# Tarekbouamer/Image-Retrieval-for-Image-Based-Localization

Measured on AMD Instinct MI355X. Metric: images/sec extract + queries/sec 1M-desc kNN, ResNet50-GeM 1024×768, higher is better.
Workload: dtype fp16

## Files before the change

### image-retrieval-for-image-based-localization_amd/cirtorch/_engine.py

```python

import contextlib
import ctypes
import os
import threading

import torch

PKG_DIR = os.path.dirname(os.path.dirname(os.path.abspath(__file__)))
LIB_PATH = os.environ.get("RR_LIB", os.path.join(PKG_DIR, "librr.so"))

RR_F32, RR_BF16, RR_F16, RR_I8 = 0, 1, 2, 3
RR_ACT_IDENTITY, RR_ACT_LEAKY = 0, 1
RR_POOL_GEM, RR_POOL_MAC, RR_POOL_SPOC = 0, 1, 2
RR_CONV_AFFINE, RR_CONV_RESIDUAL, RR_CONV_PERM32 = 1, 2, 4
RR_NHWC, RR_NCHW = 0, 1
RR_MATCH_NN, RR_MATCH_MNN, RR_MATCH_SNN, RR_MATCH_SMNN = 0, 1, 2, 3
RR_RESP_HARRIS, RR_RESP_GFTT, RR_RESP_HESSIAN, RR_RESP_DOG = 0, 1, 2, 3
RR_EPI_SAMPSON, RR_EPI_SYMMETRICAL = 0, 1
TUNE_KEYS = ("GEMM_CONFIG", "GEMM_STAGES", "GEMM_WIDE", "GEMM_ASTAT", "GEMM_XCD_MAP", "STREAM_1X1", "CONV3X3",
             "GRID_CUS", "GEMM8", "KNN_FUSED", "CONV3_PIPE", "STEM", "STREAM_XCD", "CONV3S", "WRES", "PAIR_MID",
             "WRES_RING")
globals().update(("RR_TUNE_" + name, key) for key, name in enumerate(TUNE_KEYS))
TUNE_SIZE_KEYS = {"PATCHNET_CHUNK": 32}
globals().update(("RR_TUNE_" + name, key) for name, key in TUNE_SIZE_KEYS.items())
RR_PATCHNET_HARDNET, RR_PATCHNET_SOSNET = 0, 1

_DTYPE_CODE = {torch.float32: RR_F32, torch.bfloat16: RR_BF16, torch.float16: RR_F16,
               torch.int8: RR_I8}


class ConvDesc(ctypes.Structure):
    _fields_ = [(n, ctypes.c_int) for n in ("n", "h", "w", "c_in", "ho", "wo", "c_out", "kh", "kw", "stride",
                                            "pad", "dil", "k_packed", "ldy", "act")] + \
               [("slope", ctypes.c_float), ("flags", ctypes.c_int)]


class LaunchInfo(ctypes.Structure):
    _fields_ = [("kernel", ctypes.c_char * 32), ("variant", ctypes.c_char * 48), ("grid", ctypes.c_uint),
                ("block", ctypes.c_uint), ("nslices", ctypes.c_int), ("xmap", ctypes.c_int), ("launches", ctypes.c_int)]


class Region(ctypes.Structure):
    _fields_ = [(n, ctypes.c_uint16) for n in ("y0", "x0", "h", "w")]


_vp, _i, _ll, _f, _d, _sz = ctypes.c_void_p, ctypes.c_int, ctypes.c_longlong, ctypes.c_float, ctypes.c_double, ctypes.c_size_t
_SIGS = {
    "rr_version": ([], _i),
    "rr_build_info": ([], ctypes.c_char_p),
    "rr_last_error": ([], ctypes.c_char_p),
    "rr_device_arch": ([ctypes.c_char_p, _i], _i),
    "rr_image_to_nhwc": ([_vp, _i, _i, _i, _i, ctypes.POINTER(_f), ctypes.POINTER(_f), _i, _vp, _i, _i, _vp], _i),
    "rr_conv2d_fused": ([_vp, _vp, _vp, _vp, _vp, _vp, ctypes.POINTER(ConvDesc), _i, _i, _vp], _i),
    "rr_conv1x1_pair": ([_vp, _ll, _i, _vp, _vp, _vp, _i, _vp, _vp, _vp, _vp, _vp, _i, _f, _vp, _vp, _vp, _i, _i, _f,
                         _vp, _vp, _i, _vp], _i),
    "rr_conv3x3_pair": ([_vp, _i, _i, _i, _vp, _vp, _vp, _i, _f, _vp, _vp, _vp, _i, _f, _vp, _vp, _vp, _vp, _vp, _vp, _vp, _vp, _i, _f,
                         _vp, _vp, _vp, _i, _i, _f, _vp, _vp, _vp, _i, _vp], _i),
    "rr_pack_conv_weights": ([_vp, _i, _i, _i, _i, _i, _i, _i, _vp, _i, _vp], _i),
    "rr_stem_pack_weights": ([_vp, _i, _i, _i, _i, _vp, _i, _vp], _i),
    "rr_stem_conv_pool": ([_vp, _i, _i, _i, ctypes.POINTER(_f), ctypes.POINTER(_f), _i, _vp, _vp, _vp, _i, _f, _vp,
                           _i, _i, _i, _vp], _i),
    "rr_stem_conv_pool_u8": ([_vp, _i, _i, _i, ctypes.POINTER(_f), ctypes.POINTER(_f), _i, _vp, _vp, _vp, _i, _f,
                              _vp, _i, _i, _i, _vp], _i),
    "rr_image_to_nhwc_ragged": ([_vp, _vp, _i, _i, _i, _i, _i, ctypes.POINTER(_f), ctypes.POINTER(_f), _i, _vp, _i,
                                 _i, _vp], _i),
    "rr_stem_conv_pool_ragged": ([_vp, _vp, _i, _i, _i, _i, ctypes.POINTER(_f), ctypes.POINTER(_f), _i, _vp, _vp, _vp,
                                  _i, _f, _vp, _i, _i, _i, _vp], _i),
    "rr_pad_images": ([_vp, _vp, _i, _i, _i, _i, _i, _vp, _vp, _vp], _i),
    "rr_maxpool2d": ([_vp, _i, _i, _i, _i, _i, _i, _i, _vp, _i, _i, _i, _vp], _i),
    "rr_resize_bilinear": ([_vp, _i, _i, _i, _vp, _i, _i, _d, _d, _vp], _i),
    "rr_global_pool": ([_vp, _i, _i, _i, _i, _i, _f, _f, _vp, _i, _vp], _i),
    "rr_global_pool_pdev": ([_vp, _i, _i, _i, _i, _i, _f, _vp, _f, _vp, _i, _vp], _i),
    "rr_region_pool": ([_vp, _i, _i, _i, _i, ctypes.POINTER(Region), _i, _i, _f, _vp, _i, _f, _vp, _i, _vp], _i),
    "rr_region_aggregate": ([_vp, _i, _i, _i, _i, _f, _vp, _vp], _i),
    "rr_l2n_rows": ([_vp, _i, _i, _f, _vp, _vp], _i),
    "rr_linear_rows": ([_vp, _i, _i, _vp, _vp, _i, _vp, _vp], _i),
    "rr_head_workspace_bytes": ([_i, _i], _sz),
    "rr_whiten_workspace_bytes": ([_i, _i], _sz),
    "rr_whitenapply": ([_vp, _i, _i, _vp, _vp, _i, _vp, _vp, _sz, _vp], _i),
    "rr_head_l2n_whiten_l2n": ([_vp, _i, _i, _vp, _vp, _i, _f, _vp, _vp, _vp], _i),
    "rr_knn_workspace_bytes": ([_ll, _i, _i, _i, _i, _i], _sz),
    "rr_knn_topk": ([_vp, _vp, _ll, _vp, _vp, _i, _i, _i, _i, _ll, _vp, _vp, _vp, _sz, _i, _vp], _i),
    "rr_knn_topk_checked": ([_vp, _vp, _ll, _vp, _vp, _i, _i, _i, _i, _ll, _vp, _vp, _vp, _sz, _i, _f, _vp, _vp], _i),
    "rr_topk_merge": ([_vp, _vp, _i, _i, _i, _i, _vp, _vp, _vp], _i),
    "rr_comm_unique_id": ([_vp, _i], _i),
    "rr_comm_init": ([ctypes.POINTER(_vp), _i, _vp, _i, _i], _i),
    "rr_comm_destroy": ([_vp], _i),
    "rr_topk_allgather_workspace_bytes": ([_i, _i, _i], _sz),
    "rr_topk_allgather_merge": ([_vp, _vp, _vp, _i, _i, _vp, _vp, _vp, _sz, _vp], _i),
    "rr_local_head_workspace_bytes": ([_ll, _i, _i], _sz),
# ... 182 lines not shown
```

### image-retrieval-for-image-based-localization_amd/cirtorch/_ops.py

```python

import ctypes
import os

import numpy as np
import torch

from . import _engine as E


def _st():
    return E.stream_ptr()


def _workspace(nbytes, device):
    return torch.empty(max(int(nbytes), 256), dtype=torch.uint8, device=device)


def image_to_nhwc(img, c_pad, dtype, mean=None, std=None):
    E.require_gpu(img)
    img = img.contiguous().float()
    n, c, h, w = img.shape
    out = torch.empty((n, h, w, c_pad), dtype=dtype, device=img.device)
    do = mean is not None
    m = (ctypes.c_float * 4)(*(list(mean) + [0.0] * (4 - c))[:4]) if do else (ctypes.c_float * 4)()
# ... 49 lines not shown
        return torch.empty(shape_y, dtype=dtype, device=device), torch.empty(shape_z, dtype=dtype, device=device)
    y, z = out
    E.require_gpu(y, z)
    assert tuple(y.shape) == shape_y and y.dtype == dtype and y.is_contiguous()
    assert tuple(z.shape) == shape_z and z.dtype == dtype and z.is_contiguous()
    return y, z


def conv1x1_pair(x, w3, scale3, shift3, residual, leaky3, slope3, w1, scale1, shift1, c_out, leaky1, slope1,
                 proj=None, out=None):
    E.require_gpu(x, w3, residual, w1)
    n, h, w, c = x.shape
    c_mid = w3.shape[0]
    y, z = _pair_out(out, (n, h, w, c_mid), (n, h, w, c_out), x.dtype, x.device)
    assert x.is_contiguous()
    if residual is not None:
        assert residual.shape == y.shape and residual.dtype == x.dtype and residual.is_contiguous()
        xp = wp = sp = hp = None
    else:
        xp, wp, sp, hp = proj
        E.require_gpu(xp, wp, sp, hp)
        assert xp.shape == x.shape and xp.dtype == x.dtype and xp.is_contiguous()
    E.check(E.lib().rr_conv1x1_pair(E.ptr(x), n * h * w, c, E.ptr(w3), E.ptr(scale3), E.ptr(shift3), c_mid,
                                    E.ptr(residual), E.ptr(xp), E.ptr(wp), E.ptr(sp), E.ptr(hp),
                                    E.RR_ACT_LEAKY if leaky3 else E.RR_ACT_IDENTITY, float(slope3),
                                    E.ptr(w1), E.ptr(scale1), E.ptr(shift1), c_out,
                                    E.RR_ACT_LEAKY if leaky1 else E.RR_ACT_IDENTITY, float(slope1), E.ptr(y), E.ptr(z),
                                    E.dtype_code(x.dtype), _st()), "rr_conv1x1_pair")
    return y, z


def conv3x3_pair(t1, w33, scale2, shift2, leaky2, slope2, w3, scale3, shift3, residual, leaky3, slope3,
                 w1, scale1, shift1, c_out, leaky1, slope1, proj=None, dynamic=None, conv1=None,
                 out=None):
    E.require_gpu(t1, w33, w3, residual, w1)
    n, h, w, c = t1.shape
    assert c == 64 and t1.is_contiguous() and tuple(w33.shape) == (64, 576) and tuple(w3.shape) == (256, 64)
    assert tuple(w1.shape) == (c_out, 256)
    y, z = _pair_out(out, (n, h, w, 256), (n, h, w, c_out), t1.dtype, t1.device)
    if residual is not None:
        assert residual.shape == y.shape and residual.dtype == t1.dtype and residual.is_contiguous()
        xp = wp = sp = hp = None
    else:
        xp, wp, sp, hp = proj
        E.require_gpu(xp, wp, sp, hp)
        assert tuple(xp.shape) == (n, h, w, 64) and xp.dtype == t1.dtype and xp.is_contiguous()
    act = lambda leaky: E.RR_ACT_LEAKY if leaky else E.RR_ACT_IDENTITY
    if dynamic is None:
        dynamic = os.environ.get("RR_C3PAIR_QUEUE", "1") != "0"
    queue = torch.zeros(8, dtype=torch.int32, device=t1.device) if dynamic else None
    w0, s0, h0, leaky0, slope0 = conv1 if conv1 is not None else (None, None, None, False, 0.0)
    if conv1 is not None:
        E.require_gpu(w0, s0, h0)
        assert proj is not None and tuple(w0.shape) == (64, 64)
    E.check(E.lib().rr_conv3x3_pair(E.ptr(t1), n, h, w, E.ptr(w0), E.ptr(s0), E.ptr(h0), act(leaky0), float(slope0),
                                    E.ptr(w33), E.ptr(scale2), E.ptr(shift2), act(leaky2),
                                    float(slope2), E.ptr(w3), E.ptr(scale3), E.ptr(shift3), E.ptr(residual),
                                    E.ptr(xp), E.ptr(wp), E.ptr(sp), E.ptr(hp), act(leaky3), float(slope3),
                                    E.ptr(w1), E.ptr(scale1), E.ptr(shift1), c_out, act(leaky1), float(slope1),
                                    E.ptr(y), E.ptr(z), E.ptr(queue), E.dtype_code(t1.dtype), _st()),
            "rr_conv3x3_pair")
    return y, z


def maxpool2d(x, k=3, stride=2, pad=1):
    E.require_gpu(x)
    n, h, w, c = x.shape
    ho = (h + 2 * pad - k) // stride + 1
    wo = (w + 2 * pad - k) // stride + 1
    y = torch.empty((n, ho, wo, c), dtype=x.dtype, device=x.device)
    E.check(E.lib().rr_maxpool2d(E.ptr(x), n, h, w, c, k, stride, pad, E.ptr(y), ho, wo, E.dtype_code(x.dtype),
                                 _st()), "rr_maxpool2d")
    return y


def pack_stem_weights(weight, dtype=torch.bfloat16):
    E.require_gpu(weight)
    w = weight.detach().float().contiguous()
    co, ci, kh, kw = w.shape
    out = torch.empty((co, 448), dtype=dtype, device=w.device)
    E.check(E.lib().rr_stem_pack_weights(E.ptr(w), co, ci, kh, kw, E.ptr(out), E.dtype_code(dtype), _st()),
            "rr_stem_pack_weights")
    return out


_UNIT_LUT = {}


def pixels_to_unit(x):
    lut = _UNIT_LUT.get(x.device)
    if lut is None:
        lut = torch.from_numpy(np.arange(256, dtype=np.float32) / np.float32(255.0)).to(x.device)
        _UNIT_LUT[x.device] = lut
    return lut[x.long()]
# ... 1211 lines not shown
```

### image-retrieval-for-image-based-localization_amd/cirtorch/backbones/resnet.py

```python

import os
import sys
from collections import OrderedDict
from functools import partial

import torch
import torch.nn as nn
import torch.nn.functional as F

from .. import _ops
from ..modules.abn import ABN
from .misc import ResidualBlock, make_step, run_step

CONV_PARAMS = ["weight"]
BN_PARAMS = ["weight", "bias", "running_mean", "running_var"]

_PRECISIONS = {"bf16": torch.bfloat16, "fp32": torch.float32, "float32": torch.float32, "bfloat16": torch.bfloat16,
               "fp16": torch.float16, "float16": torch.float16}


def try_index(scalar_or_list, i):
    try:
        return scalar_or_list[i]
    except TypeError:
# ... 115 lines not shown
            for blk in mod.children():
                blocks.append(blk.engine_plan(self.engine_dtype))
            plan["mods"].append(blocks)
        self._plan = plan
        return plan

    @staticmethod
    def _conv(t, st, residual=None, out=None):
        return run_step(t, st, residual, out)

    def _stem(self, plan, x, mean, std):
        if isinstance(x, (list, tuple)):
            live = [t for t in x if t is not None]
            if not live:
                raise ValueError("at least one image of the batch must be non-None")
            h = max(int(t.shape[-2]) for t in live)
            w = max(int(t.shape[-1]) for t in live)
            st = plan["stem"]
            if plan["stem_fused"] is not None:
                return _ops.stem_conv_pool_ragged(x, h, w, plan["stem_fused"], st.scale, st.shift, leaky=st.leaky,
                                                  slope=st.slope, mean=mean, std=std)
            t = _ops.image_to_nhwc_ragged(x, h, w, self.stem_cin(), self.engine_dtype, mean, std)
            return _ops.maxpool2d(self._conv(t, st), 3, 2, 1)
        if x.dtype == torch.uint8 and plan["stem_fused"] is None:
            x = _ops.pixels_to_unit(x)
        if plan["stem_fused"] is not None:
            st = plan["stem"]
            return _ops.stem_conv_pool(x, plan["stem_fused"], st.scale, st.shift, leaky=st.leaky, slope=st.slope,
                                       mean=mean, std=std)
        t = _ops.image_to_nhwc(x, self.stem_cin(), self.engine_dtype, mean, std)
        t = self._conv(t, plan["stem"])
        return _ops.maxpool2d(t, 3, 2, 1)

    def _blocks(self, t, flat, i0, i1, outs, pending=None):
        for i in range(i0, i1):
            mod_id, steps, proj = flat[i]
            nxt = flat[i + 1][1][0] if i + 1 < i1 else None
            pair = self._pairable(steps[-1], nxt)
            fuse_proj = pair and proj is not None and self._proj_fusable(proj)
            res = t if proj is None else (None if fuse_proj else self._conv(t, proj))
            block = pair and self._c3pairable(t, steps, nxt, fuse_proj)
            conv1 = block and fuse_proj and pending is None and self._conv1_fusable(t, steps[0])
            y = t
            for j, st in enumerate(steps[:-2] if block else steps[:-1]):
                if conv1:
                    break
                y = pending if (j == 0 and pending is not None) else self._conv(y, st)
            pending = None
            if block:
                mid, last = steps[-2], steps[-1]
                c1 = steps[0]
                t, pending = _ops.conv3x3_pair(y, mid.w, mid.scale, mid.shift, mid.leaky, mid.slope,
                                               last.w, last.scale, last.shift, res, last.leaky, last.slope,
                                               nxt.w, nxt.scale, nxt.shift, nxt.c_out, nxt.leaky, nxt.slope,
                                               proj=(t, proj.w, proj.scale, proj.shift) if fuse_proj else None,
                                               conv1=(c1.w, c1.scale, c1.shift, c1.leaky, c1.slope) if conv1 else None)
            elif pair:
                last = steps[-1]
                t, pending = _ops.conv1x1_pair(y, last.w, last.scale, last.shift, res, last.leaky, last.slope,
                                               nxt.w, nxt.scale, nxt.shift, nxt.c_out, nxt.leaky, nxt.slope,
                                               proj=(t, proj.w, proj.scale, proj.shift) if fuse_proj else None)
            else:
                t = self._conv(y, steps[-1], residual=res)
            if outs is not None and (i + 1 == len(flat) or flat[i + 1][0] != mod_id):
                outs["mod%d" % (mod_id + 2)] = t
        return t, pending

    def forward(self, x, normalize=None):
        plan = self._plan or self._build_plan()
        mean, std = normalize if normalize is not None else (None, None)
        outs = OrderedDict()
        flat = [(mod_id, steps, proj) for mod_id, blocks in enumerate(plan["mods"]) for steps, proj in blocks]
        t = self._stem(plan, x, mean, std)
        outs["mod1"] = t
        self._blocks(t, flat, 0, len(flat), outs)
        return OrderedDict((k, v.permute(0, 3, 1, 2)) for k, v in outs.items())

    @staticmethod
    def _proj_fusable(proj):
        return (proj.kh == 1 and proj.stride == 1 and proj.pad == 0 and proj.perm and proj.c_out == 256
                and proj.w.shape[1] == 64 and not proj.leaky)

    @staticmethod
    def _c3pairable(t, steps, nxt, fuse_proj):
        if len(steps) != 3 or os.environ.get("RR_C3PAIR", "1") == "0":
            return False
        mid, last = steps[1], steps[2]
        n, h, w, c = t.shape
        return (mid.kh == 3 and mid.kw == 3 and mid.stride == 1 and mid.pad == 1 and mid.perm and mid.c_out == 64
                and tuple(mid.w.shape) == (64, 576) and last.c_out == 256 and last.w.shape[1] == 64
                and nxt.c_out in ((64,) if fuse_proj else (64, 128)) and h % 4 == 0 and w % 32 == 0
                and n * h * w * 64 * 2 < 2 ** 31)

    @staticmethod
    def _conv1_fusable(t, st):
        return (os.environ.get("RR_C3PAIR_CONV1", "0") == "1" and st.kh == 1 and st.kw == 1 and st.stride == 1
                and st.pad == 0 and st.perm and st.c_out == 64 and tuple(st.w.shape) == (64, 64) and t.shape[-1] == 64)

    def _pairable(self, last, nxt):
        if nxt is None or self.engine_dtype == torch.float32 or os.environ.get("RR_PAIR_FUSED", "1") == "0":
            return False
        if not (last.kh == 1 and last.stride == 1 and last.perm and nxt.kh == 1 and nxt.stride == 1
                and nxt.pad == 0 and nxt.perm):
            return False
        if last.c_out == 256 and last.w.shape[1] == 64:
            return nxt.w.shape[1] == 256 and nxt.c_out in (64, 128)
        if last.c_out == 512 and last.w.shape[1] == 128 and os.environ.get("RR_PAIR_MID", "1") != "0":
            return nxt.w.shape[1] == 512 and nxt.c_out == 128
        return False
# ... 16 lines not shown
```

### image-retrieval-for-image-based-localization_amd/cirtorch/models/GF_net.py

```python

import os
from collections import OrderedDict

import numpy as np
import torch
import torch.nn as nn

from .. import _ops
from ..algos.GF_algo import globalFeatureAlgo
from ..backbones import resnet as _resnet
from ..modules.heads.global_head import globalHead
from ..modules.pools import POOLING_LAYERS
from ..utils.parallel import PackedSequence

from ..modules.utils import OUTPUT_DIM


class Normalize:

    def __init__(self, rgb_mean=(0.485, 0.456, 0.406), rgb_std=(0.229, 0.224, 0.225)):
        self.rgb_mean = list(rgb_mean)
        self.rgb_std = list(rgb_std)


# ... 10 lines not shown
        out = []
        for scale in scales:
            if scale == 1:
                out.append(img)
            else:
                out.append(PackedSequence([_ops.resize_bilinear(im, scale) for im in img]))
        return out

    def _normalizer(self):
        a = self.augment
        if a is None:
            return None
        if hasattr(a, "rgb_mean") and hasattr(a, "rgb_std"):
            return (list(a.rgb_mean), list(a.rgb_std))
        raise NotImplementedError("only normalising augment objects (rgb_mean/rgb_std) are supported at eval time")

    @property
    def pool(self):
        return self.ret_head.pool

    def meta_repr(self):
        tmp = "  (meta): dict( \n"
        for k in ("architecture", "local_whitening", "pooling", "regional", "whitening", "outputdim", "mean", "std"):
            if k in self.meta:
                tmp += "     %s: %s\n" % (k, self.meta[k])
        tmp += "  )\n"
        return tmp

    def forward(self, img=None, positive_img=None, negative_img=None, scales=[1], do_augmentaton=False,
                do_loss=False, do_prediction=True, **varargs):
        if do_loss:
            raise NotImplementedError("training (tuple loss) is out of scope for the MI355X engine")
        if isinstance(img, torch.Tensor) and img.dim() == 4 and len(scales) == 1:
            x = self.body(img, normalize=self._normalizer())
            ret_pred = self.ret_algo.inference(self.ret_head, x, [img.shape[-2:]] * img.shape[0]) \
                if do_prediction else None
            return OrderedDict([("ret_loss", None)]), OrderedDict([("ret_pred", ret_pred)])
        if isinstance(img, torch.Tensor) and img.dim() == 4:
            preds = []
            for scale in scales:
                if scale == 1:
                    xs = img
                else:
                    xf = _ops.pixels_to_unit(img) if img.dtype == torch.uint8 else img
                    xs = _ops.resize_bilinear(xf, scale)
                _, pred = self.forward(img=xs, scales=[1], do_prediction=True, do_loss=False)
                preds.append(pred["ret_pred"].unsqueeze(0))
            pred = torch.cat(preds, dim=0).permute(1, 2, 0)
            pred = nn.functional.avg_pool1d(pred, kernel_size=len(scales)).squeeze(-1)
            return OrderedDict([("ret_loss", None)]), OrderedDict([("ret_pred", pred)])
        if isinstance(img, torch.Tensor):
            if img.dtype == torch.uint8 and len(scales) > 1:
                img = _ops.pixels_to_unit(img)
            img = PackedSequence(list(img)) if img.dim() == 4 else PackedSequence([img])
        if len(scales) > 1:
            if img.dtype == torch.uint8:
                img = PackedSequence([_ops.pixels_to_unit(t) if t is not None else None for t in img])
            preds = []
            for im in self._prepare_pyramid_inputs(img, scales):
                _, pred = self.forward(img=im, scales=[1], do_prediction=True, do_loss=False)
                preds.append(pred["ret_pred"].unsqueeze(0))
            pred = torch.cat(preds, dim=0).permute(1, 2, 0)
            pred = nn.functional.avg_pool1d(pred, kernel_size=len(scales)).squeeze(-1)
            return OrderedDict([("ret_loss", None)]), OrderedDict([("ret_pred", pred)])

        images = list(img)
        x = self.body(images, normalize=self._normalizer())
        valid_size = [tuple(t.shape[-2:]) if t is not None else (0, 0) for t in images]
        if do_prediction:
            ret_pred = self.ret_algo.inference(self.ret_head, x, valid_size)
        else:
            ret_pred = None
        return OrderedDict([("ret_loss", None)]), OrderedDict([("ret_pred", ret_pred)])

    def extract(self, images, scales=(1,)):
        if not isinstance(images, torch.Tensor):
            images = PackedSequence(list(images))
        with torch.no_grad():
            _, pred = self.forward(img=images, scales=list(scales))
        return pred["ret_pred"]


def make_net(architecture="resnet50", pooling="gem", whitening=True, mean=None, std=None, precision="bf16",
             p=3.0, regional=False, regional_whitening=True, L=3):
    body = _resnet.__dict__[architecture](precision=precision)
    dim = OUTPUT_DIM[architecture]
    pname = {"gem": "GeM", "mac": "MAC", "spoc": "SPoC", "gemmp": "GeMmp"}[pooling.lower()]
    params = {"p": p, "eps": 1e-6} if pname in ("GeM", "GeMmp") else {}
    if regional:
        if pname == "GeMmp":
            params["mp"] = dim
        rwhiten = nn.Linear(dim, dim, bias=True) if regional_whitening else None
        params = {"rpool": POOLING_LAYERS[pname](**params), "whiten": rwhiten, "L": L}
        pname = "ROIpool"
    head = globalHead(pooling={"name": pname, "params": params}, normal={"name": "L2N", "params": {}}, dim=dim)
    algo = globalFeatureAlgo(loss=None, min_level=0, fpn_levels=1)
    if not whitening:
        algo._head = lambda h, x: h(x, do_whitening=False)
    augment = Normalize(mean, std) if mean is not None else None
    net = ImageRetrievalNet(body, algo, head, augment=augment)
# ... 316 lines not shown
```

### image-retrieval-for-image-based-localization_amd/csrc/rr_c3pair.hip

```cpp
#include "rr_internal.h"
#include "rr_ldsdma.h"
#include "rr_epilogue.h"
#include "rr_tilewalk.h"

#ifndef C3P_IG2
#define C3P_IG2 1
#endif

namespace rr {

namespace {

template <int K>
__device__ __forceinline__ int cwswz(int row, int chunk) {
    const int f = K == 64 ? ((row >> 1) & 7) : (row & 15);
    return row * (K * 2) + ((chunk ^ f) << 4);
}

}

struct C3PairArgs {
    const bf16_t* t1;
    const bf16_t* w0;
    const float *s0, *h0;
    const bf16_t* w33;
    const float *s33, *h33;
    const bf16_t* w3;
    const float *s3, *h3;
    const bf16_t* res;
    const bf16_t* xp;
    const bf16_t* wp;
    const float *sp, *hp;
    const bf16_t* w1;
    const float *s1, *h1;
    bf16_t* y;
    bf16_t* z;
    int* queue;
    int n, h, w;
    int act2, act3, act1, act0;
    float slope2, slope3, slope1, slope0;
};

namespace {

template <int C1, bool PROJ, typename HT, bool CONV1 = false>
__global__ void __launch_bounds__(512, 1) k_c3pair(C3PairArgs a, int tiles_w, int tiles_hw, int ntiles) {
    static_assert(!CONV1 || PROJ, "conv1 in the launch: the stage's first block only");
    constexpr int TH = 4, TW = 32, TP = TH * TW, PITCH = 40;
    constexpr int NSLOT = (TH + 2) * PITCH, NP = NSLOT / 8;
    constexpr int PCW = TW + 2;
    constexpr int FN = 4;
    constexpr int K3 = 64, C3 = 256, NK3 = K3 / 32, NR3 = C3 / 32, NF1 = C1 / 16, NK1 = C3 / 32;
    static_assert(NSLOT % 8 == 0 && PITCH % 8 == 0, "row-invariant patch swizzle");
    __shared__ __attribute__((aligned(1024))) char sPatch[NSLOT * 128];
    __shared__ __attribute__((aligned(16))) char sT2[TP * 128];
    __shared__ __attribute__((aligned(16))) char sW3[C3 * K3 * 2];
    __shared__ __attribute__((aligned(16))) char sW1[C1 * C3 * 2];
    __shared__ __attribute__((aligned(16))) char sWp[PROJ ? C3 * K3 * 2 : 16];
    __shared__ __attribute__((aligned(16))) float sS3[C3], sH3[C3], sS1[C1], sH1[C1], sS2[64], sH2[64];
    __shared__ __attribute__((aligned(16))) float sSp[PROJ ? C3 : 4], sHp[PROJ ? C3 : 4];
    __shared__ __attribute__((aligned(16))) char sW0[CONV1 ? 64 * 64 * 2 : 16];
    __shared__ __attribute__((aligned(16))) float sS0[CONV1 ? 64 : 4], sH0[CONV1 ? 64 : 4];
    __shared__ int sTile[4];

    const int tid = threadIdx.x, lane = tid & 63;
    const int wave = __builtin_amdgcn_readfirstlane(tid >> 6);
    const bool role3 = wave < 4;
    const int r16 = lane & 15, kq = lane >> 4, lrow = lane >> 3, lch = lane & 7;
    const int H = a.h, W = a.w;

    for (int i = tid; i < C3 * K3 / 8; i += 512) {
        const int r = i / (K3 / 8), c = i - r * (K3 / 8);
        *reinterpret_cast<uint4*>(sW3 + cwswz<K3>(r, c)) = reinterpret_cast<const uint4*>(a.w3)[i];
        if constexpr (PROJ) *reinterpret_cast<uint4*>(sWp + cwswz<K3>(r, c)) = reinterpret_cast<const uint4*>(a.wp)[i];
    }
    for (int i = tid; i < C1 * C3 / 8; i += 512) {
        const int r = i / (C3 / 8), c = i - r * (C3 / 8);
        *reinterpret_cast<uint4*>(sW1 + cwswz<C3>(r, c)) = reinterpret_cast<const uint4*>(a.w1)[i];
    }
    for (int i = tid; i < C3; i += 512) {
// ... 145 lines not shown
        }
        const bool leaky2 = a.act2 == RR_ACT_LEAKY;
#pragma unroll
        for (int j = 0; j < FN; ++j) {
            const int p = wpx * (TP / 2) + j * 16 + r16;
            float v[8];
            RR_BN_PAIR(acc[0][j], acc[1][j], sc, sh, v);
            if (leaky2) RR_LEAKY(8, v, a.slope2);
            uint4 o;
            RR_PACK8(HT, o, v);
            *reinterpret_cast<uint4*>(sT2 + p * 128 + (((4 * wc + kq) ^ (p & 7)) << 4)) = o;
        }
    };

    const int pw = wave - 4;
    const bool leaky3 = a.act3 == RR_ACT_LEAKY, leaky1 = a.act1 == RR_ACT_LEAKY;
    constexpr int NRQ = PROJ ? NK3 : NR3;
    auto strip_pixel = [&](int t, int k) __attribute__((always_inline)) {
        int img, oh0, ow0;
        tile_org(t, img, oh0, ow0);
        return ((long long)img * H + oh0 + (k >> 1)) * W + ow0 + (k & 1) * 16 + r16;
    };
    auto load_rq = [&](uint4 (&dst)[NRQ], long long p) __attribute__((always_inline)) {
        if constexpr (PROJ) {
            const bf16_t* ps = a.xp + p * K3 + 8 * kq;
#pragma unroll
            for (int kk = 0; kk < NK3; ++kk) dst[kk] = ld16_once(ps + kk * 32);
        } else {
            const bf16_t* rs = a.res + p * C3 + 8 * kq;
#pragma unroll
            for (int i2 = 0; i2 < NR3; ++i2) dst[i2] = ld16_once(rs + 32 * i2);
        }
    };
    auto pair_strip = [&](int k, long long p, const uint4 (&rv)[NRQ]) __attribute__((always_inline)) {
        uint4 bq[NK3];
        {
            const int q = k * 16 + r16;
#pragma unroll
            for (int kk = 0; kk < NK3; ++kk)
                bq[kk] = *reinterpret_cast<const uint4*>(sT2 + q * 128 + (((4 * kk + kq) ^ (q & 7)) << 4));
        }
        uint4 yq[NR3];
        constexpr int IG = C3P_IG2 ? 2 : 1;
#pragma unroll
        for (int i0 = 0; i0 < NR3; i0 += IG) {
            int abase = 0;
            asm volatile("" : "+v"(abase));
            f32x4_t acc3[IG][2], pacc[IG][2];
#pragma unroll
            for (int g = 0; g < IG; ++g)
#pragma unroll
                for (int hh = 0; hh < 2; ++hh) acc3[g][hh] = pacc[g][hh] = (f32x4_t){0.f, 0.f, 0.f, 0.f};
#pragma unroll
            for (int kk = 0; kk < NK3; ++kk)
#pragma unroll
                for (int g = 0; g < IG; ++g)
#pragma unroll
                    for (int hh = 0; hh < 2; ++hh) {
                        const uint4 av = *reinterpret_cast<const uint4*>(sW3 + abase + cwswz<K3>((2 * (i0 + g) + hh) * 16 + r16, kk * 4 + kq));
                        acc3[g][hh] = H16<HT>::mfma(av, bq[kk], acc3[g][hh]);
                    }
            if constexpr (PROJ) {
#pragma unroll
                for (int kk = 0; kk < NK3; ++kk)
#pragma unroll
                    for (int g = 0; g < IG; ++g)
#pragma unroll
                        for (int hh = 0; hh < 2; ++hh) {
                            const uint4 av = *reinterpret_cast<const uint4*>(sWp + abase + cwswz<K3>((2 * (i0 + g) + hh) * 16 + r16, kk * 4 + kq));
                            pacc[g][hh] = H16<HT>::mfma(av, rv[kk], pacc[g][hh]);
                        }
            }
#pragma unroll
            for (int g = 0; g < IG; ++g) {
                const int i2 = i0 + g;
                const int c = 32 * i2 + 8 * kq;
                float v[8];
                RR_BN_PAIR(acc3[g][0], acc3[g][1], sS3 + c, sH3 + c, v);
                if constexpr (PROJ) {
#pragma unroll
                    for (int r = 0; r < 4; ++r) {
                        v[r] += pacc[g][0][r] * sSp[c + r] + sHp[c + r];
                        v[4 + r] += pacc[g][1][r] * sSp[c + 4 + r] + sHp[c + 4 + r];
                    }
                } else {
                    const uint4 qv = rv[i2];
                    RR_ADD_PACKED8(HT, qv, v);
                }
                if (leaky3) RR_LEAKY(8, v, a.slope3);
                RR_PACK8(HT, yq[i2], v);
                st16_once(a.y + p * C3 + c, yq[i2]);
            }
        }
        f32x4_t zacc[NF1];
        RR_ZERO(1, zacc);
#pragma unroll
        for (int kk = 0; kk < NK1; ++kk) {
            int abase = 0;
            asm volatile("" : "+v"(abase));
#pragma unroll
            for (int o = 0; o < NF1; ++o) {
                const uint4 av = *reinterpret_cast<const uint4*>(sW1 + abase + cwswz<C3>(o * 16 + r16, kk * 4 + kq));
                zacc[o] = H16<HT>::mfma(av, yq[kk], zacc[o]);
            }
        }
#pragma unroll
        for (int o2 = 0; o2 < NF1 / 2; ++o2) {
            const int c = 32 * o2 + 8 * kq;
            float v[8];
            RR_BN_PAIR(zacc[2 * o2], zacc[2 * o2 + 1], sS1 + c, sH1 + c, v);
            if (leaky1) RR_LEAKY(8, v, a.slope1);
            uint4 o;
            RR_PACK8(HT, o, v);
            st16_once(a.z + p * C1 + c, o);
        }
    };

    if (role3) {
        uint4 areg[2][18];
#pragma unroll
        for (int i = 0; i < 2; ++i)
#pragma unroll
            for (int ks = 0; ks < 18; ++ks)
                areg[i][ks] = *reinterpret_cast<const uint4*>(a.w33 + (long long)(32 * wc + 16 * i + r16) * 576 +
// ... 19 lines not shown
        for (int s = 0; tile_id(s) >= 0; ++s) {
            const bool more = tile_id(s + 1) >= 0;
            if (wpx == 1) store_t2();
            if constexpr (CONV1) {
                if (more) convert_patch(tile_id(s + 1));
                lds_barrier();
            }
            if (more) conv();
            lds_barrier();
            if (more) {
                if (wpx == 0) store_t2();
                const int t2i = tile_id(s + 2);
                patch_dma(t2i, t2i >= 0);
                if (tid == 0) sTile[(s + 3) & 3] = t2i >= 0 ? fetch_tile(s + 3) : -1;
                vm_wait<0>();
            }
            lds_barrier();
        }
    } else {
        __builtin_amdgcn_s_setprio(1);
        uint4 rq[4][NRQ];
        load_rq(rq[0], strip_pixel(tile_id(0), pw));
        load_rq(rq[1], strip_pixel(tile_id(0), 4 + pw));
        lds_barrier();
        if constexpr (CONV1) lds_barrier();
        lds_barrier();
        lds_barrier();
        for (int s = 0; tile_id(s) >= 0; s += 2) {
            {
                const int t = tile_id(s);
                const bool n1 = tile_id(s + 1) >= 0;
                if (n1) load_rq(rq[2], strip_pixel(tile_id(s + 1), pw));
                if constexpr (CONV1) lds_barrier();
                pair_strip(pw, strip_pixel(t, pw), rq[0]);
                lds_barrier();
                if (n1) load_rq(rq[3], strip_pixel(tile_id(s + 1), 4 + pw));
                pair_strip(4 + pw, strip_pixel(t, 4 + pw), rq[1]);
                lds_barrier();
            }
            if (tile_id(s + 1) >= 0) {
                const int t = tile_id(s + 1);
                const bool n2 = tile_id(s + 2) >= 0;
                if (n2) load_rq(rq[0], strip_pixel(tile_id(s + 2), pw));
                if constexpr (CONV1) lds_barrier();
                pair_strip(pw, strip_pixel(t, pw), rq[2]);
                lds_barrier();
                if (n2) load_rq(rq[1], strip_pixel(tile_id(s + 2), 4 + pw));
                pair_strip(4 + pw, strip_pixel(t, 4 + pw), rq[3]);
                lds_barrier();
            }
        }
    }
}

}

}

using namespace rr;

extern "C" int rr_conv3x3_pair(const void* t1, int n, int h, int w, const void* w0, const float* scale0,
                               const float* shift0, int act0, float slope0, const void* w33, const float* scale2,
                               const float* shift2, int act2, float slope2, const void* w3, const float* scale3,
                               const float* shift3, const void* residual, const void* xp, const void* wp,
                               const float* scalep, const float* shiftp, int act3, float slope3, const void* w1,
                               const float* scale1, const float* shift1, int c_out, int act1, float slope1, void* y,
                               void* z, int* tile_queue, int dtype, void* stream) {
    if (dtype != RR_BF16 && dtype != RR_F16) return fail(RR_EINVAL, "rr_conv3x3_pair: dtype (bf16 / fp16)");
    if (!t1 || !w33 || !scale2 || !shift2 || !w3 || !scale3 || !shift3 || !w1 || !scale1 || !shift1 || !y || !z)
        return fail(RR_EINVAL, "rr_conv3x3_pair: null pointer");
    const bool proj = residual == nullptr;
    if (proj && (!xp || !wp || !scalep || !shiftp))
        return fail(RR_EINVAL, "rr_conv3x3_pair: either residual or the projection (xp, wp, scalep, shiftp)");
    if (c_out != 64 && c_out != 128) return fail(RR_EINVAL, "rr_conv3x3_pair: c_out 64 or 128");
    if (proj && c_out != 64) return fail(RR_EINVAL, "rr_conv3x3_pair: the projection form takes c_out = 64");
    const bool conv1 = w0 != nullptr;
    if (conv1 && (!proj || !scale0 || !shift0 || ((uintptr_t)w0 & 15)))
        return fail(RR_EINVAL, "rr_conv3x3_pair: conv1 in the launch (w0) needs the projection form, scale0, shift0");
    if (conv1 && act0 != RR_ACT_IDENTITY && act0 != RR_ACT_LEAKY) return fail(RR_EINVAL, "rr_conv3x3_pair: act0");
    if (n <= 0 || h <= 0 || w <= 0 || h % 4 || w % 32) return fail(RR_EINVAL, "rr_conv3x3_pair: h % 4, w % 32");
    if ((long long)n * h * w * 64 * 2 >= (1ll << 31)) return fail(RR_EINVAL, "rr_conv3x3_pair: t1 over 2 GiB (split the batch)");
    for (const void* p : {t1, w33, w3, residual, xp, wp, w1, (const void*)y, (const void*)z})
        if ((uintptr_t)p & 15) return fail(RR_EINVAL, "rr_conv3x3_pair: 16-byte alignment required");
    if ((uintptr_t)tile_queue & 3) return fail(RR_EINVAL, "rr_conv3x3_pair: tile_queue alignment");
    for (int act : {act2, act3, act1})
        if (act != RR_ACT_IDENTITY && act != RR_ACT_LEAKY) return fail(RR_EINVAL, "rr_conv3x3_pair: activation");
    C3PairArgs a;
    a.t1 = (const bf16_t*)t1; a.w33 = (const bf16_t*)w33; a.s33 = scale2; a.h33 = shift2;
    a.w3 = (const bf16_t*)w3; a.s3 = scale3; a.h3 = shift3; a.res = (const bf16_t*)residual;
    a.xp = (const bf16_t*)xp; a.wp = (const bf16_t*)wp; a.sp = scalep; a.hp = shiftp;
    a.w1 = (const bf16_t*)w1; a.s1 = scale1; a.h1 = shift1; a.y = (bf16_t*)y; a.z = (bf16_t*)z;
    a.n = n; a.h = h; a.w = w; a.act2 = act2; a.act3 = act3; a.act1 = act1;
    a.slope2 = slope2; a.slope3 = slope3; a.slope1 = slope1; a.queue = tile_queue;
    a.w0 = (const bf16_t*)w0; a.s0 = scale0; a.h0 = shift0; a.act0 = act0; a.slope0 = slope0;
    const int tiles_w = w / 32, tiles_hw = (h / 4) * tiles_w;
    const long long ntl = (long long)n * tiles_hw;
    if (ntl >= (1ll << 31)) return fail(RR_EINVAL, "rr_conv3x3_pair: too many tiles");
    const int cus = grid_cus();
    const int grid = persistent_grid8(ntl, cus);
    const dim3 g((unsigned)grid), b(512);
    hipStream_t s = as_stream(stream);
    auto go = [&](auto hv) {
        using H = decltype(hv);
        if (conv1) hipLaunchKernelGGL((k_c3pair<64, true, H, true>), g, b, 0, s, a, tiles_w, tiles_hw, (int)ntl);
        else if (proj) hipLaunchKernelGGL((k_c3pair<64, true, H>), g, b, 0, s, a, tiles_w, tiles_hw, (int)ntl);
        else if (c_out == 64) hipLaunchKernelGGL((k_c3pair<64, false, H>), g, b, 0, s, a, tiles_w, tiles_hw, (int)ntl);
        else hipLaunchKernelGGL((k_c3pair<128, false, H>), g, b, 0, s, a, tiles_w, tiles_hw, (int)ntl);
    };
    if (dtype == RR_F16) go(f16_t{});
    else go(bf16_t{});
    note_launch("k_c3pair", (unsigned)grid, 512, 0, 1, 1, "%d%s%s", c_out, proj ? ",proj" : "", conv1 ? ",conv1" : "");
    return check_launch("rr_conv3x3_pair");
}
```

### include/rr.h

```cpp
#ifndef RR_H_
#define RR_H_

#include <stddef.h>
#include <stdint.h>

#ifdef __cplusplus
extern "C" {
#endif

enum rr_dtype { RR_F32 = 0, RR_BF16 = 1, RR_F16 = 2, RR_I8 = 3 };
enum rr_act { RR_ACT_IDENTITY = 0, RR_ACT_LEAKY = 1 };
enum rr_pool_mode { RR_POOL_GEM = 0, RR_POOL_MAC = 1, RR_POOL_SPOC = 2 };
enum rr_conv_flags { RR_CONV_AFFINE = 1, RR_CONV_RESIDUAL = 2, RR_CONV_PERM32 = 4 };
enum rr_layout { RR_NHWC = 0, RR_NCHW = 1 };

#define RR_OK 0
#define RR_EINVAL -1
#define RR_EHIP -2
#define RR_ENOSPACE -3

int rr_version(void);
const char* rr_build_info(void);
const char* rr_last_error(void);
int rr_device_arch(char* buf, int buflen);
// ... 4 lines not shown
                     void* dst, int c_pad, int dtype, void* stream);

typedef struct rr_conv_desc {
    int n, h, w, c_in;
    int ho, wo, c_out;
    int kh, kw, stride, pad, dil;
    int k_packed;
    int ldy;
    int act;
    float slope;
    int flags;
} rr_conv_desc;

int rr_conv2d_fused(const void* x, const void* w, const float* scale, const float* shift,
                    const void* residual, void* y, const rr_conv_desc* desc,
                    int dtype, int out_dtype, void* stream);

int rr_pack_conv_weights(const float* w, int c_out, int c_in, int kh, int kw, int c_in_pad,
                         int k_packed, int perm32, void* out, int dtype, void* stream);

int rr_conv1x1_pair(const void* x, long long p, int c_in, const void* w3, const float* scale3,
                    const float* shift3, int c_mid, const void* residual, const void* xp, const void* wp,
                    const float* scalep, const float* shiftp, int act3, float slope3, const void* w1,
                    const float* scale1, const float* shift1, int c_out, int act1, float slope1, void* y,
                    void* z, int dtype, void* stream);

int rr_conv3x3_pair(const void* t1, int n, int h, int w, const void* w0, const float* scale0,
                    const float* shift0, int act0, float slope0, const void* w33, const float* scale2,
                    const float* shift2, int act2, float slope2, const void* w3, const float* scale3,
                    const float* shift3, const void* residual, const void* xp, const void* wp,
                    const float* scalep, const float* shiftp, int act3, float slope3, const void* w1,
                    const float* scale1, const float* shift1, int c_out, int act1, float slope1, void* y,
                    void* z, int* tile_queue, int dtype, void* stream);

int rr_maxpool2d(const void* x, int n, int h, int w, int c, int k, int stride, int pad,
                 void* y, int ho, int wo, int dtype, void* stream);

int rr_stem_pack_weights(const float* w, int c_out, int c_in, int kh, int kw, void* out, int dtype, void* stream);
int rr_stem_conv_pool(const float* x, int n, int h, int w, const float* mean_host, const float* std_host,
                      int do_normalize, const void* wpk, const float* scale, const float* shift, int act,
                      float slope, void* y, int hp, int wp, int dtype, void* stream);
int rr_stem_conv_pool_u8(const unsigned char* x, int n, int h, int w, const float* mean_host,
                         const float* std_host, int do_normalize, const void* wpk, const float* scale,
                         const float* shift, int act, float slope, void* y, int hp, int wp, int dtype,
                         void* stream);

int rr_image_to_nhwc_ragged(const void* const* srcs, const int* extents, int n, int c, int h, int w, int u8,
                            const float* mean_host, const float* std_host, int do_normalize,
                            void* dst, int c_pad, int dtype, void* stream);
int rr_stem_conv_pool_ragged(const void* const* srcs, const int* extents, int n, int h, int w, int u8,
                             const float* mean_host, const float* std_host, int do_normalize, const void* wpk,
                             const float* scale, const float* shift, int act, float slope, void* y, int hp, int wp,
                             int dtype, void* stream);
int rr_pad_images(const void* const* srcs, const int* extents, int n, int c, int h, int w, int elem_bytes,
                  const void* pad_value_host, void* dst, void* stream);

int rr_resize_bilinear(const float* src, int c, int h, int w, float* dst, int ho, int wo,
                       double scale_h, double scale_w, void* stream);

int rr_global_pool(const void* x, int n, int c, int hw, int layout, int mode,
                   float p, float eps, float* out, int dtype, void* stream);
int rr_global_pool_pdev(const void* x, int n, int c, int hw, int layout, int mode,
                        float p, const float* p_dev, float eps, float* out, int dtype, void* stream);

int rr_l2n_rows(const float* x, int rows, int dim, float eps, float* y, void* stream);

// ... 213 lines not shown
```

Baseline: 5608.

## Write stage-end block output at stride 2 when only the downsampling projection reads it

When a stage's final fused 3x3 pair block feeds only the next stage's stride-2 1x1 projection, and the intermediate stage output is not requested, the kernel now stores only the even rows and columns of y into a compact half-resolution buffer. The projection then runs as a stride-1 1x1 conv on that compact tensor. The GF_net retrieval path now asks the backbone for mod5 only, which makes these stages eligible. The aim is to cut y write bandwidth at stage boundaries and the strided reads in the projection, at the cost of a new kernel variant and more complex block-planning logic.

```diff
diff --git a/image-retrieval-for-image-based-localization_amd/cirtorch/_engine.py b/image-retrieval-for-image-based-localization_amd/cirtorch/_engine.py
--- a/image-retrieval-for-image-based-localization_amd/cirtorch/_engine.py
+++ b/image-retrieval-for-image-based-localization_amd/cirtorch/_engine.py
@@ -56,6 +56,8 @@
                          _vp, _vp, _i, _vp], _i),
     "rr_conv3x3_pair": ([_vp, _i, _i, _i, _vp, _vp, _vp, _i, _f, _vp, _vp, _vp, _i, _f, _vp, _vp, _vp, _vp, _vp, _vp, _vp, _vp, _i, _f,
                          _vp, _vp, _vp, _i, _i, _f, _vp, _vp, _vp, _i, _vp], _i),
+    "rr_conv3x3_pair_ys": ([_vp, _i, _i, _i, _vp, _vp, _vp, _i, _f, _vp, _vp, _vp, _i, _f, _vp, _vp, _vp, _vp, _vp, _vp, _vp, _vp, _i, _f,
+                            _vp, _vp, _vp, _i, _i, _f, _vp, _i, _vp, _vp, _i, _vp], _i),
     "rr_pack_conv_weights": ([_vp, _i, _i, _i, _i, _i, _i, _i, _vp, _i, _vp], _i),
     "rr_stem_pack_weights": ([_vp, _i, _i, _i, _i, _vp, _i, _vp], _i),
     "rr_stem_conv_pool": ([_vp, _i, _i, _i, ctypes.POINTER(_f), ctypes.POINTER(_f), _i, _vp, _vp, _vp, _i, _f, _vp,
diff --git a/image-retrieval-for-image-based-localization_amd/cirtorch/_ops.py b/image-retrieval-for-image-based-localization_amd/cirtorch/_ops.py
--- a/image-retrieval-for-image-based-localization_amd/cirtorch/_ops.py
+++ b/image-retrieval-for-image-based-localization_amd/cirtorch/_ops.py
@@ -105,14 +105,19 @@
 
 def conv3x3_pair(t1, w33, scale2, shift2, leaky2, slope2, w3, scale3, shift3, residual, leaky3, slope3,
                  w1, scale1, shift1, c_out, leaky1, slope1, proj=None, dynamic=None, conv1=None,
-                 out=None):
+                 out=None, y_stride=1):
     E.require_gpu(t1, w33, w3, residual, w1)
     n, h, w, c = t1.shape
     assert c == 64 and t1.is_contiguous() and tuple(w33.shape) == (64, 576) and tuple(w3.shape) == (256, 64)
     assert tuple(w1.shape) == (c_out, 256)
-    y, z = _pair_out(out, (n, h, w, 256), (n, h, w, c_out), t1.dtype, t1.device)
+    if y_stride not in (1, 2):
+        raise ValueError("conv3x3_pair: y_stride 1 or 2")
+    if y_stride == 2 and (residual is None or c_out != 128):
+        raise ValueError("conv3x3_pair: y_stride 2 takes the residual form with c_out = 128")
+    ys = y_stride
+    y, z = _pair_out(out, (n, h // ys, w // ys, 256), (n, h, w, c_out), t1.dtype, t1.device)
     if residual is not None:
-        assert residual.shape == y.shape and residual.dtype == t1.dtype and residual.is_contiguous()
+        assert tuple(residual.shape) == (n, h, w, 256) and residual.dtype == t1.dtype and residual.is_contiguous()
         xp = wp = sp = hp = None
     else:
         xp, wp, sp, hp = proj
@@ -126,13 +131,16 @@
     if conv1 is not None:
         E.require_gpu(w0, s0, h0)
         assert proj is not None and tuple(w0.shape) == (64, 64)
-    E.check(E.lib().rr_conv3x3_pair(E.ptr(t1), n, h, w, E.ptr(w0), E.ptr(s0), E.ptr(h0), act(leaky0), float(slope0),
-                                    E.ptr(w33), E.ptr(scale2), E.ptr(shift2), act(leaky2),
-                                    float(slope2), E.ptr(w3), E.ptr(scale3), E.ptr(shift3), E.ptr(residual),
-                                    E.ptr(xp), E.ptr(wp), E.ptr(sp), E.ptr(hp), act(leaky3), float(slope3),
-                                    E.ptr(w1), E.ptr(scale1), E.ptr(shift1), c_out, act(leaky1), float(slope1),
-                                    E.ptr(y), E.ptr(z), E.ptr(queue), E.dtype_code(t1.dtype), _st()),
-            "rr_conv3x3_pair")
+    head = (E.ptr(t1), n, h, w, E.ptr(w0), E.ptr(s0), E.ptr(h0), act(leaky0), float(slope0),
+            E.ptr(w33), E.ptr(scale2), E.ptr(shift2), act(leaky2),
+            float(slope2), E.ptr(w3), E.ptr(scale3), E.ptr(shift3), E.ptr(residual),
+            E.ptr(xp), E.ptr(wp), E.ptr(sp), E.ptr(hp), act(leaky3), float(slope3),
+            E.ptr(w1), E.ptr(scale1), E.ptr(shift1), c_out, act(leaky1), float(slope1), E.ptr(y))
+    tail = (E.ptr(z), E.ptr(queue), E.dtype_code(t1.dtype), _st())
+    if y_stride == 1:
+        E.check(E.lib().rr_conv3x3_pair(*head, *tail), "rr_conv3x3_pair")
+    else:
+        E.check(E.lib().rr_conv3x3_pair_ys(*head, y_stride, *tail), "rr_conv3x3_pair_ys")
     return y, z
 
 
diff --git a/image-retrieval-for-image-based-localization_amd/cirtorch/backbones/resnet.py b/image-retrieval-for-image-based-localization_amd/cirtorch/backbones/resnet.py
--- a/image-retrieval-for-image-based-localization_amd/cirtorch/backbones/resnet.py
+++ b/image-retrieval-for-image-based-localization_amd/cirtorch/backbones/resnet.py
@@ -171,13 +171,20 @@
         t = self._conv(t, plan["stem"])
         return _ops.maxpool2d(t, 3, 2, 1)
 
-    def _blocks(self, t, flat, i0, i1, outs, pending=None):
+    def _blocks(self, t, flat, i0, i1, outs, pending=None, want=None):
+        compact = False
         for i in range(i0, i1):
             mod_id, steps, proj = flat[i]
             nxt = flat[i + 1][1][0] if i + 1 < i1 else None
             pair = self._pairable(steps[-1], nxt)
             fuse_proj = pair and proj is not None and self._proj_fusable(proj)
-            res = t if proj is None else (None if fuse_proj else self._conv(t, proj))
+            if compact:
+                assert proj is not None and pending is not None and len(steps) == 3 and not fuse_proj
+                res = _ops.conv2d_fused(t, proj.w, 1, 1, 1, 0, proj.c_out, proj.scale, proj.shift,
+                                        leaky=proj.leaky, slope=proj.slope, perm32=proj.perm)
+                compact = False
+            else:
+                res = t if proj is None else (None if fuse_proj else self._conv(t, proj))
             block = pair and self._c3pairable(t, steps, nxt, fuse_proj)
             conv1 = block and fuse_proj and pending is None and self._conv1_fusable(t, steps[0])
             y = t
@@ -186,14 +193,19 @@
                     break
                 y = pending if (j == 0 and pending is not None) else self._conv(y, st)
             pending = None
+            stage_end = i + 1 == len(flat) or flat[i + 1][0] != mod_id
+            name = "mod%d" % (mod_id + 2)
             if block:
                 mid, last = steps[-2], steps[-1]
                 c1 = steps[0]
+                compact = (stage_end and want is not None and name not in want and res is not None
+                           and nxt.c_out == 128 and self._ys2_reader(flat[i + 1]))
                 t, pending = _ops.conv3x3_pair(y, mid.w, mid.scale, mid.shift, mid.leaky, mid.slope,
                                                last.w, last.scale, last.shift, res, last.leaky, last.slope,
                                                nxt.w, nxt.scale, nxt.shift, nxt.c_out, nxt.leaky, nxt.slope,
                                                proj=(t, proj.w, proj.scale, proj.shift) if fuse_proj else None,
-                                               conv1=(c1.w, c1.scale, c1.shift, c1.leaky, c1.slope) if conv1 else None)
+                                               conv1=(c1.w, c1.scale, c1.shift, c1.leaky, c1.slope) if conv1 else None,
+                                               y_stride=2 if compact else 1)
             elif pair:
                 last = steps[-1]
                 t, pending = _ops.conv1x1_pair(y, last.w, last.scale, last.shift, res, last.leaky, last.slope,
@@ -201,19 +213,38 @@
                                                proj=(t, proj.w, proj.scale, proj.shift) if fuse_proj else None)
             else:
                 t = self._conv(y, steps[-1], residual=res)
-            if outs is not None and (i + 1 == len(flat) or flat[i + 1][0] != mod_id):
-                outs["mod%d" % (mod_id + 2)] = t
+            if outs is not None and stage_end and (want is None or name in want):
+                assert not compact
+                outs[name] = t
+        assert not compact
         return t, pending
 
-    def forward(self, x, normalize=None):
+    STAGES = ("mod1", "mod2", "mod3", "mod4", "mod5")
+
+    def forward(self, x, normalize=None, outputs=None):
+        want = None
+        if outputs is not None:
+            if isinstance(outputs, str):
+                outputs = (outputs,)
+            want = set(outputs)
+            bad = sorted(want - set(self.STAGES), key=str)
+            if bad or not want:
+                raise ValueError("outputs: names out of %s, got %r" % (", ".join(self.STAGES), list(outputs)))
         plan = self._plan or self._build_plan()
         mean, std = normalize if normalize is not None else (None, None)
         outs = OrderedDict()
         flat = [(mod_id, steps, proj) for mod_id, blocks in enumerate(plan["mods"]) for steps, proj in blocks]
         t = self._stem(plan, x, mean, std)
-        outs["mod1"] = t
-        self._blocks(t, flat, 0, len(flat), outs)
+        if want is None or "mod1" in want:
+            outs["mod1"] = t
+        self._blocks(t, flat, 0, len(flat), outs, want=want)
         return OrderedDict((k, v.permute(0, 3, 1, 2)) for k, v in outs.items())
+
+    @staticmethod
+    def _ys2_reader(nxt_block):
+        _, steps, proj = nxt_block
+        return (os.environ.get("RR_C3PAIR_YS2", "1") != "0" and proj is not None and len(steps) == 3
+                and proj.kh == 1 and proj.kw == 1 and proj.stride == 2 and proj.pad == 0)
 
     @staticmethod
     def _proj_fusable(proj):
diff --git a/image-retrieval-for-image-based-localization_amd/cirtorch/models/GF_net.py b/image-retrieval-for-image-based-localization_amd/cirtorch/models/GF_net.py
--- a/image-retrieval-for-image-based-localization_amd/cirtorch/models/GF_net.py
+++ b/image-retrieval-for-image-based-localization_amd/cirtorch/models/GF_net.py
@@ -66,7 +66,7 @@
         if do_loss:
             raise NotImplementedError("training (tuple loss) is out of scope for the MI355X engine")
         if isinstance(img, torch.Tensor) and img.dim() == 4 and len(scales) == 1:
-            x = self.body(img, normalize=self._normalizer())
+            x = self.body(img, normalize=self._normalizer(), outputs=("mod5",))
             ret_pred = self.ret_algo.inference(self.ret_head, x, [img.shape[-2:]] * img.shape[0]) \
                 if do_prediction else None
             return OrderedDict([("ret_loss", None)]), OrderedDict([("ret_pred", ret_pred)])
@@ -99,7 +99,7 @@
             return OrderedDict([("ret_loss", None)]), OrderedDict([("ret_pred", pred)])
 
         images = list(img)
-        x = self.body(images, normalize=self._normalizer())
+        x = self.body(images, normalize=self._normalizer(), outputs=("mod5",))
         valid_size = [tuple(t.shape[-2:]) if t is not None else (0, 0) for t in images]
         if do_prediction:
             ret_pred = self.ret_algo.inference(self.ret_head, x, valid_size)
diff --git a/image-retrieval-for-image-based-localization_amd/csrc/rr_c3pair.hip b/image-retrieval-for-image-based-localization_amd/csrc/rr_c3pair.hip
--- a/image-retrieval-for-image-based-localization_amd/csrc/rr_c3pair.hip
+++ b/image-retrieval-for-image-based-localization_amd/csrc/rr_c3pair.hip
@@ -43,9 +43,25 @@
 
 namespace {
 
-template <int C1, bool PROJ, typename HT, bool CONV1 = false>
+template <typename T>
+struct YStride2 {};
+template <typename T>
+struct C3PairForm {
+    using type = T;
+    static constexpr bool ys2 = false;
+};
+template <typename T>
+struct C3PairForm<YStride2<T>> {
+    using type = T;
+    static constexpr bool ys2 = true;
+};
+
+template <int C1, bool PROJ, typename HF, bool CONV1 = false>
 __global__ void __launch_bounds__(512, 1) k_c3pair(C3PairArgs a, int tiles_w, int tiles_hw, int ntiles) {
+    using HT = typename C3PairForm<HF>::type;
+    constexpr bool YS2 = C3PairForm<HF>::ys2;
     static_assert(!CONV1 || PROJ, "conv1 in the launch: the stage's first block only");
+    static_assert(!YS2 || !PROJ, "y at stride 2: the stage's last block only");
     constexpr int TH = 4, TW = 32, TP = TH * TW, PITCH = 40;
     constexpr int NSLOT = (TH + 2) * PITCH, NP = NSLOT / 8;
     constexpr int PCW = TW + 2;
@@ -257,7 +273,14 @@
             for (int i2 = 0; i2 < NR3; ++i2) dst[i2] = ld16_once(rs + 32 * i2);
         }
     };
-    auto pair_strip = [&](int k, long long p, const uint4 (&rv)[NRQ]) __attribute__((always_inline)) {
+    auto pair_strip = [&](int t, int k, long long p, const uint4 (&rv)[NRQ]) __attribute__((always_inline)) {
+        const bool yrow = !((k >> 1) & 1);
+        long long py = p;
+        if constexpr (YS2) {
+            int img, oh0, ow0;
+            tile_org(t, img, oh0, ow0);
+            py = ((long long)img * (H >> 1) + ((oh0 + (k >> 1)) >> 1)) * (W >> 1) + ((ow0 + (k & 1) * 16 + r16) >> 1);
+        }
         uint4 bq[NK3];
         {
             const int q = k * 16 + r16;
@@ -314,7 +337,11 @@
                 }
                 if (leaky3) RR_LEAKY(8, v, a.slope3);
                 RR_PACK8(HT, yq[i2], v);
-                st16_once(a.y + p * C3 + c, yq[i2]);
+                if constexpr (YS2) {
+                    if (yrow && !(r16 & 1)) st16_once(a.y + py * C3 + c, yq[i2]);
+                } else {
+                    st16_once(a.y + p * C3 + c, yq[i2]);
+                }
             }
         }
         f32x4_t zacc[NF1];
@@ -400,10 +427,10 @@
                 const bool n1 = tile_id(s + 1) >= 0;
                 if (n1) load_rq(rq[2], strip_pixel(tile_id(s + 1), pw));
                 if constexpr (CONV1) lds_barrier();
-                pair_strip(pw, strip_pixel(t, pw), rq[0]);
+                pair_strip(t, pw, strip_pixel(t, pw), rq[0]);
                 lds_barrier();
                 if (n1) load_rq(rq[3], strip_pixel(tile_id(s + 1), 4 + pw));
-                pair_strip(4 + pw, strip_pixel(t, 4 + pw), rq[1]);
+                pair_strip(t, 4 + pw, strip_pixel(t, 4 + pw), rq[1]);
                 lds_barrier();
             }
             if (tile_id(s + 1) >= 0) {
@@ -411,10 +438,10 @@
                 const bool n2 = tile_id(s + 2) >= 0;
                 if (n2) load_rq(rq[0], strip_pixel(tile_id(s + 2), pw));
                 if constexpr (CONV1) lds_barrier();
-                pair_strip(pw, strip_pixel(t, pw), rq[2]);
+                pair_strip(t, pw, strip_pixel(t, pw), rq[2]);
                 lds_barrier();
                 if (n2) load_rq(rq[1], strip_pixel(tile_id(s + 2), 4 + pw));
-                pair_strip(4 + pw, strip_pixel(t, 4 + pw), rq[3]);
+                pair_strip(t, 4 + pw, strip_pixel(t, 4 + pw), rq[3]);
                 lds_barrier();
             }
         }
@@ -427,13 +454,13 @@
 
 using namespace rr;
 
-extern "C" int rr_conv3x3_pair(const void* t1, int n, int h, int w, const void* w0, const float* scale0,
-                               const float* shift0, int act0, float slope0, const void* w33, const float* scale2,
-                               const float* shift2, int act2, float slope2, const void* w3, const float* scale3,
-                               const float* shift3, const void* residual, const void* xp, const void* wp,
-                               const float* scalep, const float* shiftp, int act3, float slope3, const void* w1,
-                               const float* scale1, const float* shift1, int c_out, int act1, float slope1, void* y,
-                               void* z, int* tile_queue, int dtype, void* stream) {
+static int conv3x3_pair_impl(const void* t1, int n, int h, int w, const void* w0, const float* scale0,
+                             const float* shift0, int act0, float slope0, const void* w33, const float* scale2,
+                             const float* shift2, int act2, float slope2, const void* w3, const float* scale3,
+                             const float* shift3, const void* residual, const void* xp, const void* wp,
+                             const float* scalep, const float* shiftp, int act3, float slope3, const void* w1,
+                             const float* scale1, const float* shift1, int c_out, int act1, float slope1, void* y,
+                             int y_stride, void* z, int* tile_queue, int dtype, void* stream) {
     if (dtype != RR_BF16 && dtype != RR_F16) return fail(RR_EINVAL, "rr_conv3x3_pair: dtype (bf16 / fp16)");
     if (!t1 || !w33 || !scale2 || !shift2 || !w3 || !scale3 || !shift3 || !w1 || !scale1 || !shift1 || !y || !z)
         return fail(RR_EINVAL, "rr_conv3x3_pair: null pointer");
@@ -442,6 +469,10 @@
         return fail(RR_EINVAL, "rr_conv3x3_pair: either residual or the projection (xp, wp, scalep, shiftp)");
     if (c_out != 64 && c_out != 128) return fail(RR_EINVAL, "rr_conv3x3_pair: c_out 64 or 128");
     if (proj && c_out != 64) return fail(RR_EINVAL, "rr_conv3x3_pair: the projection form takes c_out = 64");
+    if (y_stride != 1 && y_stride != 2) return fail(RR_EINVAL, "rr_conv3x3_pair: y_stride 1 or 2");
+    const bool ys2 = y_stride == 2;
+    if (ys2 && (proj || c_out != 128))
+        return fail(RR_EINVAL, "rr_conv3x3_pair: y_stride 2 takes the residual form with c_out = 128");
     const bool conv1 = w0 != nullptr;
     if (conv1 && (!proj || !scale0 || !shift0 || ((uintptr_t)w0 & 15)))
         return fail(RR_EINVAL, "rr_conv3x3_pair: conv1 in the launch (w0) needs the projection form, scale0, shift0");
@@ -473,10 +504,36 @@
         if (conv1) hipLaunchKernelGGL((k_c3pair<64, true, H, true>), g, b, 0, s, a, tiles_w, tiles_hw, (int)ntl);
         else if (proj) hipLaunchKernelGGL((k_c3pair<64, true, H>), g, b, 0, s, a, tiles_w, tiles_hw, (int)ntl);
         else if (c_out == 64) hipLaunchKernelGGL((k_c3pair<64, false, H>), g, b, 0, s, a, tiles_w, tiles_hw, (int)ntl);
+        else if (ys2) hipLaunchKernelGGL((k_c3pair<128, false, YStride2<H>>), g, b, 0, s, a, tiles_w, tiles_hw, (int)ntl);
         else hipLaunchKernelGGL((k_c3pair<128, false, H>), g, b, 0, s, a, tiles_w, tiles_hw, (int)ntl);
     };
     if (dtype == RR_F16) go(f16_t{});
     else go(bf16_t{});
-    note_launch("k_c3pair", (unsigned)grid, 512, 0, 1, 1, "%d%s%s", c_out, proj ? ",proj" : "", conv1 ? ",conv1" : "");
+    note_launch("k_c3pair", (unsigned)grid, 512, 0, 1, 1, "%d%s%s%s", c_out, proj ? ",proj" : "", conv1 ? ",conv1" : "",
+                ys2 ? ",ys2" : "");
     return check_launch("rr_conv3x3_pair");
 }
+
+extern "C" int rr_conv3x3_pair(const void* t1, int n, int h, int w, const void* w0, const float* scale0,
+                               const float* shift0, int act0, float slope0, const void* w33, const float* scale2,
+                               const float* shift2, int act2, float slope2, const void* w3, const float* scale3,
+                               const float* shift3, const void* residual, const void* xp, const void* wp,
+                               const float* scalep, const float* shiftp, int act3, float slope3, const void* w1,
+                               const float* scale1, const float* shift1, int c_out, int act1, float slope1, void* y,
+                               void* z, int* tile_queue, int dtype, void* stream) {
+    return conv3x3_pair_impl(t1, n, h, w, w0, scale0, shift0, act0, slope0, w33, scale2, shift2, act2, slope2, w3, scale3,
+                             shift3, residual, xp, wp, scalep, shiftp, act3, slope3, w1, scale1, shift1, c_out, act1,
+                             slope1, y, 1, z, tile_queue, dtype, stream);
+}
+
+extern "C" int rr_conv3x3_pair_ys(const void* t1, int n, int h, int w, const void* w0, const float* scale0,
+                                  const float* shift0, int act0, float slope0, const void* w33, const float* scale2,
+                                  const float* shift2, int act2, float slope2, const void* w3, const float* scale3,
+                                  const float* shift3, const void* residual, const void* xp, const void* wp,
+                                  const float* scalep, const float* shiftp, int act3, float slope3, const void* w1,
+                                  const float* scale1, const float* shift1, int c_out, int act1, float slope1, void* y,
+                                  int y_stride, void* z, int* tile_queue, int dtype, void* stream) {
+    return conv3x3_pair_impl(t1, n, h, w, w0, scale0, shift0, act0, slope0, w33, scale2, shift2, act2, slope2, w3, scale3,
+                             shift3, residual, xp, wp, scalep, shiftp, act3, slope3, w1, scale1, shift1, c_out, act1,
+                             slope1, y, y_stride, z, tile_queue, dtype, stream);
+}
diff --git a/include/rr.h b/include/rr.h
--- a/include/rr.h
+++ b/include/rr.h
@@ -60,6 +60,14 @@
                     const float* scalep, const float* shiftp, int act3, float slope3, const void* w1,
                     const float* scale1, const float* shift1, int c_out, int act1, float slope1, void* y,
                     void* z, int* tile_queue, int dtype, void* stream);
+
+int rr_conv3x3_pair_ys(const void* t1, int n, int h, int w, const void* w0, const float* scale0,
+                       const float* shift0, int act0, float slope0, const void* w33, const float* scale2,
+                       const float* shift2, int act2, float slope2, const void* w3, const float* scale3,
+                       const float* shift3, const void* residual, const void* xp, const void* wp,
+                       const float* scalep, const float* shiftp, int act3, float slope3, const void* w1,
+                       const float* scale1, const float* shift1, int c_out, int act1, float slope1, void* y,
+                       int y_stride, void* z, int* tile_queue, int dtype, void* stream);
 
 int rr_maxpool2d(const void* x, int n, int h, int w, int c, int k, int stride, int pad,
                  void* y, int ho, int wo, int dtype, void* stream);
```

Measured after the change: 5640 (median of 6 runs). Within noise of the previous version (+0.6%).
